# fukangl/SMG-multimodal-grasping

Hardware: AMD Instinct MI355X
Metric: affordance fwd+bwd passes/sec (16-rot 224^2 RGB-D) (higher is better)
Workload: dtype f32; 1 GPU; 16 rot x 224^2 (S=640): fwd + Huber + bwd + Adam per GPU per step; reinforcement_net style 0; 17 trunk passes; fp32; leg=headline, rotations=16, input_size=640, parallelism=dp1

## Files before the change

### smg-multimodal-grasping_amd/csrc/backward.hip

```cpp
#include "engine.h"

int do_backward(smg_engine* e, const smg_net* net, const float* dq, hipStream_t st, int phases, bool elem_head) {
    if (!e->have_fwd) return fail(-22, "smg_backward without a preceding smg_forward");
    if (!net->grads) return fail(-22, "net.grads is NULL");
    if (phases == 2 && !e->bw_phase0_done)
        return fail(-22, "smg_backward_phase(1) must follow smg_backward_phase(0) of the same forward");
    if ((phases & 1) && e->bw_phase0_done)
        return fail(-22, "smg_backward / smg_backward_phase(0) while the second half of a two-phase backward is still due (run phase 1 or a new forward)");
    const Layout& L = *e->L;
    const TrunkRef& T = L.trunk[e->f_trunk];
    const HeadRef& Hd = L.head[e->f_head];
    const int NS = e->f_streams, NP = e->f_pairs;
    const float* P = net->params;
    float* Gr = net->grads;
    const Plane p4 = e->p_blk[3];
    const bool ph_a = phases & 1, ph_b = phases & 2;
    if (ph_a) {
        for (int r = 0; r < kStatRep; ++r) HIP_OK(hipMemsetAsync(e->bstat + (size_t)r * kStatRepStride, 0, 2 * e->bstat_span * sizeof(double), st));
    }
    const bool split16 = e->prec == 0 && kSplitOp == 3;
    if (ph_a && split16) HIP_OK(hipMemsetAsync(e->gamax, 0, (size_t)e->gamax_words * sizeof(unsigned), st));
    const hipStream_t s2 = (e->prof || e->serialize) ? st : e->side;
    auto fork = [&](hipEvent_t ev) -> int {
        HIP_OK(hipEventRecord(ev, st));
// ... 183 lines not shown
            };
            PREC_DISPATCH(e, if (int rc = go(PTAG)) return rc);
        }
        return 0;
    };
    auto debug_stop = [&]() -> int {
        launch_reduce2(e, s2, tiles.drain());
        HIP_OK(hipEventRecord(e->ev_end, s2));
        HIP_OK(hipStreamWaitEvent(st, e->ev_end, 0));
        HIP_OK(hipMemsetAsync(e->dbscr, 0, (size_t)kDbRep * e->db_total * sizeof(float), st));
        if (int rc = walk_status(e)) return rc;
        e->have_fwd = false; e->bw_phase0_done = false; e->prof_stage = -1;
        return 0;
    };
    const bool pooled_tail = e->prec == 0 && e->f_stem1 && !e->stem_plane_tail && (NS > 4 || e->deterministic);
    for (int b = ph_a ? 3 : 0; b >= (ph_b ? 0 : 1); --b) {
        e->prof_stage = b;
        const Plane pl = e->p_blk[b];
        const int Ct = kBlockCtot[b];
        if (e->dbg_stop == b * 100 + 50) return debug_stop();
        if (b == 0 && pooled_tail) {
            StemMomArgs a;
            a.img = e->img4; a.pi = e->p_img; a.ps = e->p_stem; a.part = e->mom_part;
            a.tiles_x = stem_mom_tiles_x(e->p_stem); a.n_tiles = stem_mom_tiles(e->p_stem); a.tiles_per_wg = kMomTilesPerWg;
            if (fork(e->ev_misc)) return -5;
            e->prof_stage = -1;
            launch_kernel(e, stem_moments_kernel, dim3(e->mom_groups, NS), dim3(256), 0, s2, K_OTHER, 0, 0, false, a);
            launch_kernel(e, stem_moments_sum_kernel, dim3((kMomOut + 255) / 256, NS), dim3(256), 0, s2, K_OTHER, 0, 0, false,
                          (const float*)e->mom_part, e->mom_groups, e->mom);
            e->prof_stage = b;
// ... 117 lines not shown
                    p.ldg = kBottleneck; p.pa = pl; p.KA = kBottleneck; p.N = cs;
                    p.mbuf = e->X[b]; p.ldm = Ct;
                    p.msum = fsum(e, e->st_X[b]); p.msq = fsq(e, e->st_X[b]); p.mstride = Ct; p.mtab = stat_table(e, e->sx_tab[b], e->max_streams, Ct);
                    p.dst = e->G[b]; p.ldd = Ct;
                    p.o1 = b1(e, e->st_X[b]); p.o2 = b2(e, e->st_X[b]); p.ostride = Ct; p.rep_stride = e->db_total; p.eps = kEps;
                    launch_gemm(e, st, p, dim3(NS * pl.HWp / Cfg::BM, (cs + Cfg::BN - 1) / Cfg::BN), K_D1, 2.0 * NS * pl.HW * cs * kBottleneck * p.nseg,
                                ESZ(e) * NS * pl.HW * ((double)p.nseg * kBottleneck + 3.0 * cs));
                };
                PREC_DISPATCH(e, if (pl.HWp % 128 == 0) run(GemmCfg<128, 64, 32, 2, 2, 1, true>{}, PTAG); else run(CfgP64x64{}, PTAG));
            }
            if (e->dbg_stop == b * 100 + i) return debug_stop();
        }
        if (b > 0) {
            const Plane pp = e->p_blk[b - 1];
            const int Cp = kBlockCtot[b - 1], C0 = kBlockCin[b];
            {
                int chunk, cps;
                pick_chunk(pl, NS, (C0 / 128) * (Cp / 128), chunk, cps);
                auto go = [&](auto ptag) -> int {
                BwdWeightP<MC<CfgW128x128, decltype(ptag)::value>, W_POOL, C_IDENT, 1, true, decltype(ptag)::value> p{};
                p.gbuf = e->G[b]; p.ldg = Ct; p.gcoff = 0; p.xbuf = e->X[b]; p.ldx = Ct; p.xcoff = 0; p.pa = pl; p.MA = C0;
                p.xsum = fsum(e, e->st_X[b]); p.xsq = fsq(e, e->st_X[b]); p.xstride = Ct;
                p.s1 = b1(e, e->st_X[b]); p.s2 = b2(e, e->st_X[b]); p.sstride = Ct; p.scoff = 0; p.agamma = nullptr;
                p.bbuf = e->X[b - 1]; p.ldb = Cp; p.pb = pp; p.NB = Cp;
                p.bsum = fsum(e, e->st_X[b - 1]); p.bsq = fsq(e, e->st_X[b - 1]); p.bstride = Cp;
                p.bgamma = P + T.tnorm[b - 1].w; p.bbeta = P + T.tnorm[b - 1].b; p.eps = kEps;
                p.chunk = chunk; p.chunks_per_stream = cps; p.n_chunks = NS * cps;
                p.dw = Gr + T.tconv[b - 1].w; p.ldw_out = Cp;
                if (fork(e->ev_misc)) return -5;
                const dim3 grid(C0 / 128, Cp / 128, NS * cps);
                return launch_wgrad(e, s2, p, grid, K_TW, 2.0 * NS * pl.HW * Cp * C0,
                                    ESZ(e) * NS * (2.0 * pl.HW * C0 + (double)pp.HW * Cp), 1, C_IDENT, tiles, tiles.place_alone(wgrad_partial_floats(p, grid)));
                };
                PREC_DISPATCH(e, if (int rc = go(PTAG)) return rc);
            }
            if (pp.H != 2 * pl.H || pp.W != 2 * pl.W) {
                PREC_DISPATCH(e, launch_kernel(e, zero_uncovered_kernel<PREC>, dim3(256, NS), dim3(256), 0, st, K_OTHER, 0, 0, false,
                                               (void*)e->G[b - 1], Cp, pp, 2 * pl.H, 2 * pl.W, Cp));
            }
            {
                auto run = [&](auto tag, auto ptag) {
                using Cfg = MC<decltype(tag), decltype(ptag)::value>;
                BwdDataP<Cfg, false, E_UNPOOL, true, decltype(ptag)::value> p{};
                p.gbuf = e->G[b]; p.ldg = Ct; p.gcoff = 0; p.xbuf = e->X[b]; p.ldx = Ct; p.xcoff = 0; p.pa = pl; p.KA = C0;
                p.xsum = fsum(e, e->st_X[b]); p.xsq = fsq(e, e->st_X[b]); p.xstride = Ct;
                p.s1 = b1(e, e->st_X[b]); p.s2 = b2(e, e->st_X[b]); p.sstride = Ct; p.scoff = 0; p.agamma = nullptr;
                p.wp = e->packed_u + e->pk_td[b - 1]; p.K8tot = C0 / 8; p.ldn = Cp; p.wcol0 = 0; p.N = Cp;
                p.mbuf = e->X[b - 1]; p.ldm = Cp; p.mcoff = 0; p.pm = pp;
                p.msum = fsum(e, e->st_X[b - 1]); p.msq = fsq(e, e->st_X[b - 1]); p.mstride = Cp;
                p.egamma = P + T.tnorm[b - 1].w; p.ebeta = P + T.tnorm[b - 1].b;
                p.dst = e->G[b - 1]; p.ldd = Cp; p.dcoff = 0;
                p.o1 = b1(e, e->st_X[b - 1]); p.o2 = b2(e, e->st_X[b - 1]); p.ostride = Cp; p.ocoff = 0;
                p.dbeta = e->dbscr + e->db_toff[b - 1]; p.dgamma = e->dbscr + e->db_toff[b - 1] + Cp; p.rep_stride = e->db_total; p.eps = kEps;
                launch_gemm(e, st, p, dim3(NS * pl.HWp / Cfg::BM, Cp / Cfg::BN), K_TD, 2.0 * NS * pl.HW * Cp * C0,
                            ESZ(e) * NS * (2.0 * pl.HW * C0 + 2.0 * pp.HW * Cp));
            };
            PREC_DISPATCH(e, run(CfgP64x128{}, PTAG));
            }
        }
    }
    e->prof_stage = -1;
    if (ph_b && pooled_tail) {
        const Plane p1 = e->p_blk[0];
        StemTailArgs a;
        a.G1 = e->G[0]; a.X1 = e->X[0]; a.ld1 = kBlockCtot[0]; a.p1 = p1;
        a.xsum = fsum(e, e->st_X[0]); a.xsq = fsq(e, e->st_X[0]); a.xstride = kBlockCtot[0];
        a.SA = b1(e, e->st_X[0]); a.SB = b2(e, e->st_X[0]); a.sstride = kBlockCtot[0];
        a.argmax = e->argmax; a.stemv = e->stemv;
        a.ssum = fsum(e, e->st_stem); a.ssq = fsq(e, e->st_stem); a.ps = e->p_stem;
        a.gamma = P + T.norm0.w; a.eps = kEps;
        a.img = e->img4; a.pi = e->p_img;
        a.o1 = b1(e, e->st_stem); a.o2 = b2(e, e->st_stem);
// ... 77 lines not shown
```

### smg-multimodal-grasping_amd/csrc/elem.cuh

```cuda
#pragma once
#include "gemm.cuh"

namespace smg {

struct PrepArgs {
    const float* images_nchw;
    const double* heightmaps;
    int hm, pad, S;
    double mean, stdv;
    const int* stream_image;
    const float* stream_affine;
    const int* stream_rotated;
    float* img4;
    float* img1;
    int HWp;
    const double* masks;
    const int* stream_mask_a;
    const int* stream_mask_b;
};

__device__ __forceinline__ float lin_coord(int i, int S, float step) {
    return (i < S / 2) ? fmaf(step, (float)i, -1.f) : fmaf(-step, (float)(S - 1 - i), 1.f);
}

// ... 1232 lines not shown
#pragma unroll
    for (int o = 32; o > 0; o >>= 1) vmax = fmaxf(vmax, __shfl_xor(vmax, o));
    if ((t & 63) == 0) red[t >> 6] = vmax;
    __syncthreads();
    vmax = fmaxf(fmaxf(red[0], red[1]), fmaxf(red[2], red[3]));
    ActScale sc{1.f, 1.f};
    if (vmax > 0.f) sc = scale_of_max(__float_as_uint(vmax));
    if (t == 0) a.binv[(int64_t)n * (a.pl.HWp / kScaleBlock) + blockIdx.x] = sc.inv;
    char* ob = reinterpret_cast<char*>(a.out + d2_stream_units(n, a.pl.HWp));
#pragma unroll
    for (int k = 0; k < 8; ++k) {
        const Split4 s = split4<3>(mul4(gv[k], sc.s));
        const int64_t at = ((int64_t)(cs >> 1) * a.pl.HWp + r0 + 8 * k) * 16 + (cs & 1) * 8;
        *reinterpret_cast<uint2*>(ob + at) = s.p[0];
        *reinterpret_cast<uint2*>(ob + at + (int64_t)kD2K8 * a.pl.HWp * 16) = s.p[1];
    }
}

struct DbSegD { int64_t grad_off; int scr_off; int n; };
static __global__ void db_flush_kernel(const DbSegD* segs, float* scr, int rep_stride, int reps, float* grads,
                                       const double* stem1, const double* stem2, int ns, float* dbeta0, float* dgamma0) {
    if (blockIdx.y == gridDim.y - 1) {
        if (blockIdx.x == 0 && threadIdx.x < 128 && stem1) {
            const int q = threadIdx.x >> 6, c = threadIdx.x & 63;
            double v = 0.0;
            for (int n = 0; n < ns; ++n) v += stat_get(q ? stem2 : stem1, (int64_t)n * 64 + c);
            (q ? dgamma0 : dbeta0)[c] += (float)v;
        }
        return;
    }
// ... 238 lines not shown
```

### smg-multimodal-grasping_amd/csrc/engine.h

```cpp
#pragma once
#include <hip/hip_runtime.h>

#include <algorithm>
#include <cmath>
#include <cstdio>
#include <cstdlib>
#include <cstring>
#include <string>
#include <type_traits>
#include <vector>

#include "../../include/smg_hip.h"
#include "elem.cuh"
#include "scene.cuh"
#include "gemm.cuh"
#include "halo.cuh"
#include "ws.cuh"
#include "wsw.cuh"
#include "plan.h"

using namespace smg;

int smg_fail(int code, const std::string& msg);
static inline int fail(int code, const std::string& msg) { return smg_fail(code, msg); }
// ... 43 lines not shown

struct StatArr { int64_t off; int stride; };

struct smg_engine {
    int device = 0, S = 0, max_streams = 0, max_pairs = 0, head_out = 1;
    Plane p_img, p_stem, p_blk[4];
    int OH = 1, OW = 1;
    const Layout* L = nullptr;

    float* img4 = nullptr; float* stem = nullptr; float* X[4] = {}; float* Bt = nullptr;
    std::vector<int64_t> bt_off[4];
    unsigned char* argmax = nullptr;
    float* F = nullptr; float* H1 = nullptr;
    float* G[4] = {}; float* GS[kRing] = {}; float* D2[kRing] = {}; float* part = nullptr; int64_t part_floats = 0;
    float* DY2 = nullptr; float* D2S[kRing] = {};
    hipStream_t side = nullptr; hipEvent_t ev_gs[kRing] = {}, ev_d2[kRing] = {}, ev_side[kRing] = {}, ev_misc = nullptr, ev_end = nullptr; float* DY0 = nullptr; float* DH1 = nullptr; float* DF = nullptr;
    double* fstat = nullptr; int64_t fstat_span = 0;
    double* bstat = nullptr; int64_t bstat_span = 0;
    float* dbscr = nullptr; int db_total = 0; int db_off[4][24] = {}; int db_toff[3] = {}; struct DbSeg* d_dbseg = nullptr; int n_dbseg = 0;
    StatArr st_stem, st_X[4], st_F, st_H1; std::vector<StatArr> st_Bt[4];
    u32x4* packed_u = nullptr; int64_t packed_units = 0;
    float* packed_f = nullptr; int64_t packed_floats = 0;
    PackDesc* d_pack = nullptr; std::vector<PackDesc> h_pack[3]; std::vector<PackDesc> h_pack_head[3];
    int pack_stride = 0, bnupd_stride = 0, n_bnupd = 0;
    int64_t pk_conv0 = 0, pk_conv0_1 = 0, pk_head0 = 0, pk_hd0 = 0, pk_head1 = 0;
    std::vector<int64_t> pk_c1[4], pk_d1[4], pk_g3f[4], pk_g3d[4], pk_hf[4], pk_hd[4]; int64_t pk_t[3] = {}, pk_td[3] = {};
    int max_pack = 0;
    float* asc = nullptr; ActScaleDesc* d_asc = nullptr; int n_asc = 0;
    unsigned* gamax = nullptr; int64_t gamax_words = 0;
    float* stab = nullptr; int64_t stab_floats = 0;
    int64_t sx_tab[4] = {}, sb_tab[4][24] = {}, sf_tab = 0;
    BnUpdDesc* d_bnupd = nullptr;
    bool have_fwd = false; int f_trunk = 0, f_head = 0, f_streams = 0, f_pairs = 0;
    bool bw_phase0_done = false;
    bool f_dense_dq = false;
    int head_bwd = 0;
    bool f_stem1 = false;
    int* d_stream_image = nullptr; int* d_stream_rot = nullptr; int* d_pair_a = nullptr; int* d_pair_b = nullptr;
    int* d_seq_t = nullptr; int* d_seq_h = nullptr; int* d_user_ptr = nullptr; int* d_user_pair = nullptr; int* d_user_slot = nullptr;
    float* d_affine = nullptr;
    float* scene_val = nullptr; int* scene_idx = nullptr; int scene_tiles = 0;
    double* scene_lpart = nullptr;
    double* scene_gpart = nullptr; int* scene_cnt = nullptr;
    int* d_stage = nullptr; int* h_stage[2] = {}; hipEvent_t ev_stage[2] = {}; int stage_ints = 0, stage_turn = 0;
    int so_image = 0, so_rot = 0, so_pa = 0, so_pb = 0, so_seq_t = 0, so_seq_h = 0, so_uptr = 0, so_upair = 0, so_uslot = 0, so_aff = 0, so_ma = 0, so_mb = 0, so_adam = 0;
    bool capturing = false; int* h_stage_g = nullptr; hipEvent_t ev_graph = nullptr, ev_gin = nullptr; hipStream_t gstream = nullptr; struct StepGraph* step_graph = nullptr;
    int64_t workspace_bytes = 0;
    int n_cu = 256;
    int prec = 0;
    bool serialize = false;
    bool deterministic = false;
    bool generic3x3 = false, generic_c1 = false, generic_w1 = false, stem_plane_tail = false;
    float* stemv = nullptr; float* mom_part = nullptr; double* mom = nullptr; int mom_groups = 0;
    int dbg_stop = -1;
    float* dbg_gsnap = nullptr; int64_t dbg_gsnap_floats = 0;
    bool prof = false; std::vector<ProfRec> recs; std::vector<hipEvent_t> ev_pool;
    double prof_ms[5][K_COUNT] = {}; int64_t prof_n[5][K_COUNT] = {}; double prof_flops[5][K_COUNT] = {}; double prof_bytes[5][K_COUNT] = {}; int prof_stage = -1;
    int launch_rc = 0;
};

constexpr int kMomTilesPerWg = 8;
static inline int stem_mom_tiles_x(const Plane& ps) { return (ps.W + kMomT - 1) / kMomT; }
static inline int stem_mom_tiles(const Plane& ps) { return stem_mom_tiles_x(ps) * ((ps.H + kMomT - 1) / kMomT); }
static inline int stem_mom_groups(const Plane& ps) { return (stem_mom_tiles(ps) + kMomTilesPerWg - 1) / kMomTilesPerWg; }

static Plane make_plane(int H, int W) {
    Plane p; p.H = H; p.W = W; p.HW = H * W;
// ... 204 lines not shown
```

### smg-multimodal-grasping_amd/csrc/engine.hip

```cpp
#include "engine.h"

static thread_local std::string g_err;
int smg_fail(int code, const std::string& msg) { g_err = msg; return code; }

static int engine_build(smg_engine* e) {
    const Layout& L = *e->L;
    const int NS = e->max_streams, NP = e->max_pairs;
    const int S = e->S;
    const int H1 = (S - 1) / 2 + 1, H2 = (H1 - 1) / 2 + 1;
    e->p_img = make_plane(S, S);
    e->p_stem = make_plane(H1, H1);
    int h = H2;
    for (int b = 0; b < 4; ++b) { e->p_blk[b] = make_plane(h, h); h /= 2; }
    e->OH = e->OW = e->p_blk[3].H - kHeadKernel + 1;
    if (e->OH < 1) return fail(-22, "input_size too small for the 20x20 value head");

    if (getenv("SMG_SERIALIZE")) e->serialize = true;
    const int cross = getenv("SMG_CROSSCHECK") ? atoi(getenv("SMG_CROSSCHECK")) : 0;
    e->generic3x3 = cross & 1; e->generic_c1 = cross & 2; e->generic_w1 = cross & 4; e->stem_plane_tail = cross & 8;

    ALLOC(e->img4, (int64_t)NS * e->p_img.HWp * 4);
    ALLOC(e->stem, (int64_t)NS * e->p_stem.HWp * 64);
    ALLOC(e->DY0, (int64_t)NS * e->p_stem.HWp * 64);
    ALLOC(e->argmax, (int64_t)NS * e->p_blk[0].HWp * 64);
    e->stemv = e->DY0;
    e->mom_groups = stem_mom_groups(e->p_stem);
    ALLOC(e->mom_part, (int64_t)NS * e->mom_groups * kMomVals);
    ALLOC(e->mom, (int64_t)NS * kMomOut);
    int64_t bt_total = 0;
    for (int b = 0; b < 4; ++b) {
        ALLOC(e->X[b], (int64_t)NS * e->p_blk[b].HWp * kBlockCtot[b]);
        ALLOC(e->G[b], (int64_t)NS * e->p_blk[b].HWp * kBlockCtot[b]);
        for (int i = 0; i < kBlockLayers[b]; ++i) {
            e->bt_off[b].push_back(bt_total);
            bt_total += (int64_t)NS * e->p_blk[b].HWp * kBottleneck;
        }
    }
    ALLOC(e->Bt, bt_total);
    for (int k = 0; k < kRing; ++k) {
        ALLOC(e->D2[k], (int64_t)NS * e->p_blk[0].HWp * kBottleneck);
        ALLOC(e->GS[k], (int64_t)NS * e->p_blk[0].HWp * kGrowth);
        ALLOC(e->D2S[k], (int64_t)NS * (e->p_blk[0].HWp / kScaleBlock));
        HIP_OK(hipEventCreateWithFlags(&e->ev_gs[k], hipEventDisableTiming));
        HIP_OK(hipEventCreateWithFlags(&e->ev_d2[k], hipEventDisableTiming));
        HIP_OK(hipEventCreateWithFlags(&e->ev_side[k], hipEventDisableTiming));
    }
    ALLOC(e->DY2, (int64_t)NS * e->p_blk[0].HWp * kBottleneck);
    e->scene_tiles = (int)(((int64_t)(S / 2) * (S / 2) + kSceneTile - 1) / kSceneTile);
    ALLOC(e->scene_val, (int64_t)kSceneMaps * e->scene_tiles);
    ALLOC(e->scene_idx, (int64_t)kSceneMaps * e->scene_tiles);
    ALLOC(e->scene_lpart, (int64_t)kSceneMaps * e->OH * e->OW);
    ALLOC(e->scene_gpart, (int64_t)kSceneMaps * e->OH * e->OW * 3);
    ALLOC(e->scene_cnt, (int64_t)kSceneMaps * e->OH * e->OW);
    HIP_OK(hipEventCreateWithFlags(&e->ev_misc, hipEventDisableTiming));
    HIP_OK(hipEventCreateWithFlags(&e->ev_end, hipEventDisableTiming));
    HIP_OK(hipStreamCreateWithFlags(&e->side, hipStreamNonBlocking));
    e->part_floats = (int64_t)24 << 20;
    for (int b = 0; b < 4; ++b) {
        const Plane& pl = e->p_blk[b];
        for (int ts : {halo_tile(pl), 8})
            e->part_floats = std::max(e->part_floats, w3_partial_floats(w3_tiling(pl, ts, NS, INT64_MAX).groups, NS));
    }
    ALLOC(e->part, e->part_floats);
    ALLOC(e->F, (int64_t)NP * e->p_blk[3].HWp * 2 * kFeat);
    ALLOC(e->DF, (int64_t)NP * e->p_blk[3].HWp * 2 * kFeat);
    ALLOC(e->H1, (int64_t)NP * e->p_blk[3].HWp * kHeadMid);
    ALLOC(e->DH1, (int64_t)NP * e->p_blk[3].HWp * kHeadMid);

    int64_t off = 0;
    auto carve = [&](int n, int stride) { StatArr s{off, stride}; off += (int64_t)n * stride; return s; };
// ... 71 lines not shown
                int64_t g2 = 0, g3 = 0;
                const int64_t hf = add_units(v, d.c2.w, kGrowth, kBottleneck, PK_HF, 9 * kBottleneck, kGrowth, kSplitOp);
                const int64_t hd = add_units(v, d.c2.w, kGrowth, kBottleneck, PK_HD, 9 * kGrowth, kBottleneck, kSplitOp);
                if (e->generic3x3) {
                    g2 = add_units(v, d.c2.w, kGrowth, kBottleneck, PK_3F, 9 * kBottleneck, kGrowth, kSplitOp);
                    g3 = add_units(v, d.c2.w, kGrowth, kBottleneck, PK_3D, 9 * kGrowth, kBottleneck);
                }
                if (t == 0) {
                    e->pk_c1[b].push_back(a1); e->pk_d1[b].push_back(a1d);
                    e->pk_g3f[b].push_back(g2); e->pk_g3d[b].push_back(g3); e->pk_hf[b].push_back(hf); e->pk_hd[b].push_back(hd);
                }
            }
            if (b < 3) {
                e->pk_t[b] = add_units(v, T.tconv[b].w, T.tconv[b].cout, T.tconv[b].cin, PK_T1, T.tconv[b].cin, T.tconv[b].cout, kSplitOp);
                e->pk_td[b] = add_units(v, T.tconv[b].w, T.tconv[b].cout, T.tconv[b].cin, PK_D1, T.tconv[b].cout, T.tconv[b].cin);
            }
        }
    }
    const int64_t trunk_pku = pku, trunk_pkf = pkf;
    for (int hd = 0; hd < 3; ++hd) {
        pku = trunk_pku; pkf = trunk_pkf;
        const HeadRef& H = L.head[hd];
        std::vector<PackDesc>& v = e->h_pack_head[hd];
        e->pk_head0 = add_units(v, H.c0.w, kHeadMid, 2 * kFeat, PK_T1, 2 * kFeat, kHeadMid, kSplitOp);
        e->pk_hd0 = add_units(v, H.c0.w, kHeadMid, 2 * kFeat, PK_D1, kHeadMid, 2 * kFeat);
        e->pk_head1 = add_f32(v, H.c1.w, e->head_out, kHeadMid, PK_HEAD, H.c1.count());
    }
    e->packed_units = pku + 4096;
    e->packed_floats = pkf;
    ALLOC(e->packed_u, e->packed_units);
// ... 186 lines not shown
    {
        int cus = 0;
        if (hipDeviceGetAttribute(&cus, hipDeviceAttributeMultiprocessorCount, device) == hipSuccess && cus > 0) e->n_cu = cus;
    }
    int r = engine_build(e);
    if (r) { smg_engine_destroy(e); return r; }
    *out = e;
    return 0;
}

void smg_engine_destroy(smg_engine* e) {
    if (!e) return;
    (void)hipSetDevice(e->device);
    (void)hipDeviceSynchronize();
    void* ptrs[] = {e->img4, e->stem, e->DY0, e->argmax, e->X[0], e->X[1], e->X[2], e->X[3], e->G[0], e->G[1], e->G[2], e->G[3],
                    e->Bt, e->DY2, e->part, e->F, e->DF, e->H1, e->DH1, e->fstat, e->bstat, e->dbscr, e->d_dbseg, e->asc, e->d_asc, e->gamax, e->packed_u, e->packed_f, e->stab, e->d_pack, e->d_bnupd,
                    e->d_stage, e->scene_val, e->scene_idx, e->scene_lpart, e->scene_gpart, e->scene_cnt, e->mom_part, e->mom};
    for (void* p : ptrs) if (p) (void)hipFree(p);
    if (e->dbg_gsnap) (void)hipFree(e->dbg_gsnap);
    step_graph_drop(e);
    if (e->h_stage_g) (void)hipHostFree(e->h_stage_g);
    if (e->ev_graph) (void)hipEventDestroy(e->ev_graph);
    if (e->ev_gin) (void)hipEventDestroy(e->ev_gin);
    if (e->gstream) (void)hipStreamDestroy(e->gstream);
    for (int k = 0; k < 2; ++k) { if (e->h_stage[k]) (void)hipHostFree(e->h_stage[k]); if (e->ev_stage[k]) (void)hipEventDestroy(e->ev_stage[k]); }
    for (int k = 0; k < kRing; ++k) {
        if (e->D2[k]) (void)hipFree(e->D2[k]);
        if (e->GS[k]) (void)hipFree(e->GS[k]);
        if (e->D2S[k]) (void)hipFree(e->D2S[k]);
        if (e->ev_gs[k]) (void)hipEventDestroy(e->ev_gs[k]); if (e->ev_d2[k]) (void)hipEventDestroy(e->ev_d2[k]); if (e->ev_side[k]) (void)hipEventDestroy(e->ev_side[k]);
    }
    if (e->ev_misc) (void)hipEventDestroy(e->ev_misc);
    if (e->ev_end) (void)hipEventDestroy(e->ev_end);
    if (e->side) (void)hipStreamDestroy(e->side);
    for (auto& r : e->recs) { (void)hipEventDestroy(r.a); (void)hipEventDestroy(r.b); }
    for (auto ev : e->ev_pool) (void)hipEventDestroy(ev);
    delete e;
}

int64_t smg_engine_workspace_bytes(const smg_engine* e) { return e ? e->workspace_bytes : 0; }

int smg_engine_geometry(const smg_engine* e, int H[6], int HWp[6]) {
    if (!e) return fail(-22, "engine is NULL");
    const Plane* pl[6] = {&e->p_img, &e->p_stem, &e->p_blk[0], &e->p_blk[1], &e->p_blk[2], &e->p_blk[3]};
    for (int i = 0; i < 6; ++i) { H[i] = pl[i]->H; HWp[i] = pl[i]->HWp; }
    return 0;
}

// ... 576 lines not shown
```

### smg-multimodal-grasping_amd/csrc/gemm.cuh

```cuda
#pragma once
#include <hip/hip_runtime.h>
#include <stdint.h>

#include <type_traits>

#include "wgrad_plan.h"

namespace smg {
constexpr int kDmaFlyDgrad = 2, kDmaFlyGroup = 1;
constexpr int kPdFwdSmall = 3;
constexpr int kPdFwdBig = 2;
constexpr int kPdDgrad = 2;
constexpr int kPdDgradBig = 2;
constexpr int kPdWgrad = 3;
constexpr int kPdDgradGroup = 1;
constexpr int kFwdBigMinWaves = 3;
}

namespace smg {

typedef float f32x16 __attribute__((ext_vector_type(16)));
typedef __bf16 bf16x8 __attribute__((ext_vector_type(8)));
typedef short s16x4 __attribute__((ext_vector_type(4)));
typedef unsigned u32x4 __attribute__((ext_vector_type(4)));
// ... 1167 lines not shown
    int N;
    const void* mbuf; int ldm; int mcoff; Plane pm;
    const double* msum; const double* msq; int mstride; StatTab mtab;
    const float* egamma; const float* ebeta;
    void* dst; int ldd; int dcoff;
    double* o1; double* o2; int ostride; int ocoff;
    float* dbeta; float* dgamma; int rep_stride;
    float eps;
    TileMap tm;
    static constexpr int kSwizzle = 1;
    static constexpr int kPrefetch = (Cfg::TM * Cfg::TN <= 2) ? kPdDgrad : kPdDgradBig;
    static constexpr int kDmaFly = kAUnit ? kDmaFlyDgrad : 0;
    static constexpr bool kSegmented = false;
    static constexpr bool kHasPrologue = true;
    static constexpr bool kEarlyFetch = EMODE != E_UNPOOL;
    static constexpr int kMinWaves = (PREC == 0 && EMODE == E_UNPOOL) ? 3 : 1;

    static constexpr bool kFast = !SHIFT3 && !AFF;
    static constexpr bool kEarly = EMODE != E_UNPOOL;
    static constexpr bool kWide = GT::size == 2;
    struct Ctx {
        int n, m0, n0; bool whole;
        float ginv[2];
        float xv[(kEarly && !kWide) ? Cfg::TM : 1][(kEarly && !kWide) ? Cfg::TN : 1][16];
        float gold[(kEarly && !kWide && EMODE == E_ACCUM) ? Cfg::TM : 1][(kEarly && !kWide && EMODE == E_ACCUM) ? Cfg::TN : 1][16];
        rawq_t<XT> xq[(kEarly && kWide) ? Cfg::TM : 1][(kEarly && kWide) ? Cfg::TN : 1][4];
        rawq_t<GT> gq[(kEarly && kWide && EMODE == E_ACCUM) ? Cfg::TM : 1][(kEarly && kWide && EMODE == E_ACCUM) ? Cfg::TN : 1][4];
    };
    struct ARow { int y, x; bool valid; unsigned off; };
    struct DRow {};
    using KPrm = KPrm0;
    using KFin = KPrm0;
    __device__ KPrm k_fetch(const Ctx&, int, int) const { return KPrm{}; }
    __device__ KFin k_finish(const Ctx&, const KPrm&, int, int, const float*) const { return KFin{}; }

    __host__ __device__ int param_floats() const { return 4 * KA + 5 * Cfg::BN; }

    __device__ void d_init(const Ctx&, DRow&, int) const {}
    __device__ void d_next(const Ctx&, DRow&) const {}
    __device__ bool init_ctx(Ctx& c, const VBlock& vb) const {
        int mt = vb.x, nt = vb.y;
        if (tm.nM && !tile_decode(tm, vb.x, mt, nt)) return false;
        c.m0 = sgpr(mt * Cfg::BM);
        c.n0 = sgpr(nt * Cfg::BN);
        c.n = sgpr(c.m0 / pa.HWp);
        const int pbase = c.m0 - c.n * pa.HWp;
        if (pbase >= pa.HW) return false;
        c.whole = kEarly && pbase + Cfg::BM <= pa.HW && (c.n0 + Cfg::BN <= N || (N & 31) == 0);
        c.ginv[0] = c.ginv[1] = 1.f;
        if constexpr (kOp == 3) {
            static_assert(Cfg::BM == kScaleBlock || (Cfg::BM == 2 * kScaleBlock && Cfg::WM == 2), "a wave's rows lie in one scale block");
            const float* bi = binv + (int64_t)c.n * (pa.HWp / kScaleBlock) + pbase / kScaleBlock;
            const float wi = pack_inv_scale(wp);
            c.ginv[0] = bi[0] * wi;
            c.ginv[1] = (Cfg::BM > kScaleBlock ? bi[1] : bi[0]) * wi;
        }
        return true;
    }
    __device__ UnitSrc a_unit_src(const Ctx& c, int kt, int piece, int k8, int row) const {
        return UnitSrc{static_cast<const u32x4*>(gbuf) + d2_stream_units(c.n, pa.HWp), kWholeBuf,
                       16u * (unsigned)((piece * kD2K8 + k8) * pa.HWp + row), 16u * (unsigned)(kt * Cfg::K8 * pa.HWp + (c.m0 - c.n * pa.HWp))};
    }
    __device__ u32x4 a_unit(const Ctx& c, int kt, int piece, int k8, int row) const {
        const UnitSrc u = a_unit_src(c, kt, piece, k8, row);
        return bload_u4(u.base, u.bytes, u.voff, u.soff);
    }
    __device__ u32x4 a_unit_d(const Ctx&, int, int, int, int) const { return u32x4{}; }
    __device__ void early_fetch(Ctx& c) const {
        if constexpr (kEarly) {
            if (c.whole) {
                const int t = threadIdx.x, lane = t & 63, wmn = (t >> 6) % (Cfg::WM * Cfg::WN), l31 = lane & 31, half = lane >> 5;
                const int wm0 = (wmn / Cfg::WN) * Cfg::TM * 32, wn0 = (wmn % Cfg::WN) * Cfg::TN * 32;
                if constexpr (kWide) {
    #pragma unroll
                    for (int i = 0; i < Cfg::TM; ++i)
    #pragma unroll
// ... 31 lines not shown
        }
    }
    __device__ void init_params(const Ctx& c, float* sp) const {
        const double inv = 1.0 / (double)pa.HW;
        for (int k = threadIdx.x; xbuf && k < KA; k += 256) {
            float mean, invstd;
            bn_moments(xsum, xsq, (int64_t)c.n * xstride + xcoff + k, inv, eps, mean, invstd);
            const float g = agamma ? agamma[k] : 1.f;
            const float q1 = (float)(stat_get(s1, (int64_t)c.n * sstride + scoff + k) * inv);
            const float q2 = (float)(stat_get(s2, (int64_t)c.n * sstride + scoff + k) * inv);
            sp[k] = g * invstd;
            sp[KA + k] = q1;
            sp[2 * KA + k] = mean;
            sp[3 * KA + k] = invstd * q2;
        }
        float* ep = sp + 4 * KA;
        const double minv = 1.0 / (double)pm.HW;
        for (int j = threadIdx.x; j < Cfg::BN; j += 256) {
            const int col = c.n0 + j;
            float mean = 0.f, invstd = 0.f, g = 0.f, b = 0.f;
            if (col < N) {
                tab_or_moments(mtab, c.n, mcoff + col, msum, msq, (int64_t)c.n * mstride + mcoff + col, minv, eps, mean, invstd);
                g = egamma[col];
                b = ebeta[col];
            }
            ep[j] = g * invstd;
            ep[Cfg::BN + j] = b;
            ep[2 * Cfg::BN + j] = mean;
            ep[3 * Cfg::BN + j] = invstd;
            ep[4 * Cfg::BN + j] = g;
        }
// ... 47 lines not shown
        if (!xbuf) return o.v[0];
        return affine2(o.v[0], o.v[1], sp + a_chan(kt, q), KA);
    }
    __device__ ARaw a_fetch_d(const Ctx&, const DRow&, int, int, int) const { return ARaw{}; }
    __device__ UnitSrc b_unit_src(const Ctx& c, int kt, int piece, int k8, int r) const {
        return UnitSrc{wp, kWholeBuf, 16u * (unsigned)((piece * K8tot + k8) * ldn + r), 16u * (unsigned)(kt * Cfg::K8 * ldn + wcol0 + c.n0)};
    }
    __device__ BRaw b_unit(const Ctx& c, int kt, int piece, int k8, int r) const {
        const UnitSrc u = b_unit_src(c, kt, piece, k8, r);
        return bload_u4(u.base, u.bytes, u.voff, u.soff);
    }
    __device__ u32x4 b_unit_xform(const Ctx&, const BRaw& o, int) const { return o; }
    __device__ void epilogue(const Ctx& c, f32x16 (&acc)[Cfg::TM][Cfg::TN], float* smem, float* sp, bool active) const {
        const int t = threadIdx.x, lane = t & 63, wmn = (t >> 6) % (Cfg::WM * Cfg::WN), l31 = lane & 31, half = lane >> 5;
        const int wm0 = (wmn / Cfg::WN) * Cfg::TM * 32, wn0 = (wmn % Cfg::WN) * Cfg::TN * 32;
        const float* ep = sp + 4 * KA;
#ifdef SMG_TRACE_EPI
        unsigned long long* etr = (g_smg_trace && threadIdx.x == 0) ? g_smg_trace + 8 * (size_t)blockIdx.x : nullptr;
        if (etr) etr[0] = smg_stamp();
#endif
        float v[2][Cfg::TN];
#pragma unroll
        for (int j = 0; j < Cfg::TN; ++j) v[0][j] = v[1][j] = 0.f;
        if constexpr (kOp == 3) {
            const float gi = wm0 >= kScaleBlock ? c.ginv[1] : c.ginv[0];
#pragma unroll
            for (int i = 0; i < Cfg::TM; ++i)
#pragma unroll
                for (int j = 0; j < Cfg::TN; ++j)
#pragma unroll
                    for (int r = 0; r < 16; ++r) acc[i][j][r] *= gi;
// ... 78 lines not shown
                                o[k] = pg_[k] * dy;
                                s0[k] += dy;
                                s1[k] += dy * ((xv4[k] - pm_[k]) * pi_[k]);
                            }
                            stq<GT>(dst, (pix0 + (d >> 1) * pm.W + (d & 1)) * ldd + dcoff + c.n0 + cq0, make_float4(o[0], o[1], o[2], o[3]));
                        }
                        quad_transpose4(s0[0], s0[1], s0[2], s0[3]);
                        quad_transpose4(s1[0], s1[1], s1[2], s1[3]);
                        v[0][j] += (s0[0] + s0[1]) + (s0[2] + s0[3]);
                        v[1][j] += (s1[0] + s1[1]) + (s1[2] + s1[3]);
                    }
            } else
#pragma unroll
            for (int i = 0; i < Cfg::TM; ++i) {
                constexpr int NL = (EMODE == E_UNPOOL) ? 4 : 1;
                constexpr int RB = (EMODE == E_UNPOOL) ? 8 : 16;
#pragma unroll
                for (int rb = 0; rb < 16; rb += RB) {
                    float xv[RB][NL], gold[RB];
                    int pix0[RB];
                    bool ok[RB];
#pragma unroll
                    for (int q = 0; q < RB; ++q) {
                        const int r = rb + q;
                        const int row = SMG_ACC_ROW(wm0, i, r, half);
                        const int p = pbase + row;
                        ok[q] = active && p < pa.HW && cok;
                        gold[q] = 0.f;
                        if constexpr (EMODE == E_UNPOOL) {
                            const int y = p / pa.W, x = p - y * pa.W;
                            pix0[q] = c.n * pm.HWp + (2 * y) * pm.W + 2 * x;
// ... 432 lines not shown
        if (etr) { etr[3] = smg_stamp(); asm volatile("s_waitcnt vmcnt(0)" ::: "memory"); etr[4] = smg_stamp(); }
#endif
    }
};

enum { W_ONE = 0, W_THREE = 1, W_POOL = 2, W_STEM = 3, W_STEM1 = 4 };

template <class Cfg_, int BMODE, int CMAP, int PD_ = kPdWgrad, bool AFF = true, int PREC = 0, bool F32IO_ = false>
struct BwdWeightP {
    using Cfg = Cfg_;
    static_assert(!Cfg::AT, "weight-gradient form");
    static constexpr bool F32IO = F32IO_ || BMODE == 3 || BMODE == 4;
    using GT = typename std::conditional<F32IO, e_f32, grd_t<PREC>>::type;
    using XT = typename std::conditional<F32IO, e_f32, act_t<PREC>>::type;
    static_assert(GT::size == XT::size, "one slot geometry");
    static constexpr int kOp = (!AFF && BMODE == 0) ? bwd_op(PREC) : bwd_op_plain(PREC), kAE = 16 / GT::size, kBE = 16 / XT::size, GSZ = GT::size, XSZ = XT::size;
    static constexpr bool kARawCopy = !AFF && kAE == 8;
    static constexpr bool kAUnit = !AFF && BMODE == 0 && kOp == 3;
    static constexpr bool kH = kOp == 3;
    const float* binv;
    const float* basc;
    const void* gbuf; int ldg; int gcoff;
    const void* xbuf; int ldx; int xcoff;
    Plane pa; int MA;
    const double* xsum; const double* xsq; int xstride;
    const double* s1; const double* s2; int sstride; int scoff;
    const float* agamma;
    const void* bbuf; int ldb; Plane pb; int NB;
    const double* bsum; const double* bsq; int bstride; StatTab btab;
    const float* bgamma; const float* bbeta;
    float eps;
    int chunk, chunks_per_stream, n_chunks;
    float* dw; int ldw_out;
// ... 44 lines not shown
        c.m0 = sgpr((tile % gx) * Cfg::BM);
        c.n0 = sgpr((tile / gx) * Cfg::BN);
        c.tap = sgpr(z / n_chunks);
        const int ci = z - c.tap * n_chunks;
        c.n = sgpr(ci / chunks_per_stream);
        c.p0 = sgpr((ci - c.n * chunks_per_stream) * chunk);
        if (c.p0 >= pa.HW) return false;
        int len = pa.HWp - c.p0;
        len = len < chunk ? len : chunk;
        c.kt = sgpr(len / Cfg::BK);
        c.cur_inv = 1.f;
        if constexpr (kAUnit) c.cur_inv = binv[(int64_t)c.n * (pa.HWp / kScaleBlock) + c.p0 / kScaleBlock];
        return true;
    }
    __device__ u32x4 a_unit_d(const Ctx& c, int kt, int piece, int k8, int kr) const {
        return bload_u4(static_cast<const u32x4*>(gbuf) + d2_stream_units(c.n, pa.HWp), 16u * (unsigned)(2 * kD2K8 * pa.HWp),
                        16u * (unsigned)((piece * kD2K8 + k8) * pa.HWp + kr), 16u * (unsigned)(c.p0 + kt * Cfg::BK));
    }
    __device__ u32x4 a_unit(const Ctx&, int, int, int, int) const { return u32x4{}; }
    __device__ void k_hook(Ctx& c, int kt, f32x16 (&acc)[Cfg::TM][Cfg::TN], const float* sp) const {
        if constexpr (kAUnit) {
            const int nx = (kt + 1) * Cfg::BK;
            if (nx % kScaleBlock || kt + 1 >= c.kt) return;
            const float inv = sp[kInvAt + nx / kScaleBlock];
            if (inv != c.cur_inv) {
                const float f = c.cur_inv * __uint_as_float((254u << 23) - __float_as_uint(inv));
#pragma unroll
                for (int i = 0; i < Cfg::TM; ++i)
#pragma unroll
                    for (int j = 0; j < Cfg::TN; ++j)
#pragma unroll
                        for (int r = 0; r < 16; ++r) acc[i][j][r] *= f;
// ... 263 lines not shown
```

Before: 64.54 passes/s.

## Precompute transition-layer gradient units once and share across wgrad and dgrad

Adds a trans_units_kernel that applies the BN-backward affine to the transition gradient once per block, computes per-row-block scales, and writes split 16-bit unit tiles. The pooled transition weight-gradient and unpool data-gradient GEMMs then read these precomputed units instead of each recomputing the affine from fp32 G/X. This replaces reading fp32 G and X twice with one extra kernel pass plus a compact buffer. It adds an event to guard reuse of the TU buffer across blocks and raises min waves for the non-affine unpool path.

```diff
diff --git a/smg-multimodal-grasping_amd/csrc/backward.hip b/smg-multimodal-grasping_amd/csrc/backward.hip
--- a/smg-multimodal-grasping_amd/csrc/backward.hip
+++ b/smg-multimodal-grasping_amd/csrc/backward.hip
@@ -221,6 +221,7 @@
         return 0;
     };
     const bool pooled_tail = e->prec == 0 && e->f_stem1 && !e->stem_plane_tail && (NS > 4 || e->deterministic);
+    bool tu_busy = false;
     for (int b = ph_a ? 3 : 0; b >= (ph_b ? 0 : 1); --b) {
         e->prof_stage = b;
         const Plane pl = e->p_blk[b];
@@ -368,14 +369,31 @@
         if (b > 0) {
             const Plane pp = e->p_blk[b - 1];
             const int Cp = kBlockCtot[b - 1], C0 = kBlockCin[b];
+            const bool t_units = split16 && !e->trans_on_the_fly && NS > 4;
+            if (t_units) {
+                if (tu_busy) HIP_OK(hipStreamWaitEvent(st, e->ev_tu, 0));
+                TransUnitsArgs a{};
+                a.g = e->G[b]; a.x = e->X[b]; a.ld = Ct; a.pl = pl; a.xtab = stat_table(e, e->sx_tab[b], e->max_streams, Ct);
+                a.s1 = b1(e, e->st_X[b]); a.s2 = b2(e, e->st_X[b]); a.sstride = Ct;
+                a.out = reinterpret_cast<u32x4*>(e->TU); a.binv = e->TUS;
+                const dim3 grid(pl.HWp / kScaleBlock, NS);
+                const double bytes = 4.0 * NS * pl.HW * 3 * C0;
+                if (C0 == 128) launch_kernel(e, trans_units_kernel<128>, grid, dim3(256), 0, st, K_OTHER, 0, bytes, false, a);
+                else if (C0 == 256) launch_kernel(e, trans_units_kernel<256>, grid, dim3(512), 0, st, K_OTHER, 0, bytes, false, a);
+                else launch_kernel(e, trans_units_kernel<512>, grid, dim3(1024), 0, st, K_OTHER, 0, bytes, false, a);
+            }
             {
                 int chunk, cps;
                 pick_chunk(pl, NS, (C0 / 128) * (Cp / 128), chunk, cps);
-                auto go = [&](auto ptag) -> int {
-                BwdWeightP<MC<CfgW128x128, decltype(ptag)::value>, W_POOL, C_IDENT, 1, true, decltype(ptag)::value> p{};
-                p.gbuf = e->G[b]; p.ldg = Ct; p.gcoff = 0; p.xbuf = e->X[b]; p.ldx = Ct; p.xcoff = 0; p.pa = pl; p.MA = C0;
+                auto go = [&](auto ptag, auto afftag) -> int {
+                constexpr bool AFF = decltype(afftag)::value;
+                BwdWeightP<MC<CfgW128x128, decltype(ptag)::value>, W_POOL, C_IDENT, 1, AFF, decltype(ptag)::value> p{};
+                p.pa = pl; p.MA = C0;
+                if constexpr (AFF) {
+                p.gbuf = e->G[b]; p.ldg = Ct; p.gcoff = 0; p.xbuf = e->X[b]; p.ldx = Ct; p.xcoff = 0;
                 p.xsum = fsum(e, e->st_X[b]); p.xsq = fsq(e, e->st_X[b]); p.xstride = Ct;
                 p.s1 = b1(e, e->st_X[b]); p.s2 = b2(e, e->st_X[b]); p.sstride = Ct; p.scoff = 0; p.agamma = nullptr;
+                } else { p.gbuf = e->TU; p.xbuf = nullptr; p.binv = e->TUS; p.basc = asc_trans(e, b - 1); }
                 p.bbuf = e->X[b - 1]; p.ldb = Cp; p.pb = pp; p.NB = Cp;
                 p.bsum = fsum(e, e->st_X[b - 1]); p.bsq = fsq(e, e->st_X[b - 1]); p.bstride = Cp;
                 p.bgamma = P + T.tnorm[b - 1].w; p.bbeta = P + T.tnorm[b - 1].b; p.eps = kEps;
@@ -386,20 +404,28 @@
                 return launch_wgrad(e, s2, p, grid, K_TW, 2.0 * NS * pl.HW * Cp * C0,
                                     ESZ(e) * NS * (2.0 * pl.HW * C0 + (double)pp.HW * Cp), 1, C_IDENT, tiles, tiles.place_alone(wgrad_partial_floats(p, grid)));
                 };
-                PREC_DISPATCH(e, if (int rc = go(PTAG)) return rc);
+                if (t_units) {
+                    if (int rc = go(std::integral_constant<int, 0>{}, std::false_type{})) return rc;
+                    HIP_OK(hipEventRecord(e->ev_tu, s2));
+                    tu_busy = true;
+                } else PREC_DISPATCH(e, if (int rc = go(PTAG, std::true_type{})) return rc);
             }
             if (pp.H != 2 * pl.H || pp.W != 2 * pl.W) {
                 PREC_DISPATCH(e, launch_kernel(e, zero_uncovered_kernel<PREC>, dim3(256, NS), dim3(256), 0, st, K_OTHER, 0, 0, false,
                                                (void*)e->G[b - 1], Cp, pp, 2 * pl.H, 2 * pl.W, Cp));
             }
             {
-                auto run = [&](auto tag, auto ptag) {
+                auto run = [&](auto tag, auto ptag, auto afftag) {
                 using Cfg = MC<decltype(tag), decltype(ptag)::value>;
-                BwdDataP<Cfg, false, E_UNPOOL, true, decltype(ptag)::value> p{};
-                p.gbuf = e->G[b]; p.ldg = Ct; p.gcoff = 0; p.xbuf = e->X[b]; p.ldx = Ct; p.xcoff = 0; p.pa = pl; p.KA = C0;
+                constexpr bool AFF = decltype(afftag)::value;
+                BwdDataP<Cfg, false, E_UNPOOL, AFF, decltype(ptag)::value> p{};
+                p.pa = pl; p.KA = C0;
+                if constexpr (AFF) {
+                p.gbuf = e->G[b]; p.ldg = Ct; p.gcoff = 0; p.xbuf = e->X[b]; p.ldx = Ct; p.xcoff = 0;
                 p.xsum = fsum(e, e->st_X[b]); p.xsq = fsq(e, e->st_X[b]); p.xstride = Ct;
                 p.s1 = b1(e, e->st_X[b]); p.s2 = b2(e, e->st_X[b]); p.sstride = Ct; p.scoff = 0; p.agamma = nullptr;
-                p.wp = e->packed_u + e->pk_td[b - 1]; p.K8tot = C0 / 8; p.ldn = Cp; p.wcol0 = 0; p.N = Cp;
+                } else { p.gbuf = e->TU; p.xbuf = nullptr; p.binv = e->TUS; }
+                p.wp = e->packed_u + (AFF ? e->pk_td[b - 1] : e->pk_tdu[b - 1]); p.K8tot = C0 / 8; p.ldn = Cp; p.wcol0 = 0; p.N = Cp;
                 p.mbuf = e->X[b - 1]; p.ldm = Cp; p.mcoff = 0; p.pm = pp;
                 p.msum = fsum(e, e->st_X[b - 1]); p.msq = fsq(e, e->st_X[b - 1]); p.mstride = Cp;
                 p.egamma = P + T.tnorm[b - 1].w; p.ebeta = P + T.tnorm[b - 1].b;
@@ -409,7 +435,8 @@
                 launch_gemm(e, st, p, dim3(NS * pl.HWp / Cfg::BM, Cp / Cfg::BN), K_TD, 2.0 * NS * pl.HW * Cp * C0,
                             ESZ(e) * NS * (2.0 * pl.HW * C0 + 2.0 * pp.HW * Cp));
             };
-            PREC_DISPATCH(e, run(CfgP64x128{}, PTAG));
+            if (t_units) run(CfgP64x128{}, std::integral_constant<int, 0>{}, std::false_type{});
+            else PREC_DISPATCH(e, run(CfgP64x128{}, PTAG, std::true_type{}));
             }
         }
     }
diff --git a/smg-multimodal-grasping_amd/csrc/elem.cuh b/smg-multimodal-grasping_amd/csrc/elem.cuh
--- a/smg-multimodal-grasping_amd/csrc/elem.cuh
+++ b/smg-multimodal-grasping_amd/csrc/elem.cuh
@@ -1270,6 +1270,65 @@
         const int64_t at = ((int64_t)(cs >> 1) * a.pl.HWp + r0 + 8 * k) * 16 + (cs & 1) * 8;
         *reinterpret_cast<uint2*>(ob + at) = s.p[0];
         *reinterpret_cast<uint2*>(ob + at + (int64_t)kD2K8 * a.pl.HWp * 16) = s.p[1];
+    }
+}
+
+struct TransUnitsArgs {
+    const float* g; const float* x; int ld;
+    Plane pl;
+    StatTab xtab;
+    const double* s1; const double* s2; int sstride;
+    u32x4* out; float* binv;
+};
+template <int C>
+static __global__ __launch_bounds__(2 * C) void trans_units_kernel(const TransUnitsArgs a) {
+    constexpr int NW = 2 * C / 64, K8 = C / 8;
+    __shared__ float prm[4 * C];
+    __shared__ float red[NW];
+    const int n = blockIdx.y, t = threadIdx.x;
+    const int cs = t >> 3, rr = t & 7;
+    const int r0 = blockIdx.x * kScaleBlock + rr;
+    float4 gv[8], xv[8];
+#pragma unroll
+    for (int k = 0; k < 8; ++k) {
+        const int r = r0 + 8 * k;
+        const int64_t pix = (int64_t)n * a.pl.HWp + (r < a.pl.HW ? r : 0);
+        gv[k] = ld4(a.g + pix * a.ld + 4 * cs);
+        xv[k] = ld4(a.x + pix * a.ld + 4 * cs);
+    }
+    if (t < C) {
+        const double inv = 1.0 / (double)a.pl.HW;
+        const float invstd = a.xtab.invstd[(int64_t)n * a.xtab.ld + t];
+        prm[t] = invstd;
+        prm[C + t] = (float)(stat_get(a.s1, (int64_t)n * a.sstride + t) * inv);
+        prm[2 * C + t] = a.xtab.mean[(int64_t)n * a.xtab.ld + t];
+        prm[3 * C + t] = invstd * (float)(stat_get(a.s2, (int64_t)n * a.sstride + t) * inv);
+    }
+    __syncthreads();
+    float vmax = 0.f;
+#pragma unroll
+    for (int k = 0; k < 8; ++k) {
+        const float4 o = r0 + 8 * k < a.pl.HW ? affine2(gv[k], xv[k], prm + 4 * cs, C) : zero4();
+        gv[k] = o;
+        vmax = fmaxf(fmaxf(vmax, fmaxf(fabsf(o.x), fabsf(o.y))), fmaxf(fabsf(o.z), fabsf(o.w)));
+    }
+#pragma unroll
+    for (int o = 32; o > 0; o >>= 1) vmax = fmaxf(vmax, __shfl_xor(vmax, o));
+    if ((t & 63) == 0) red[t >> 6] = vmax;
+    __syncthreads();
+    vmax = red[0];
+#pragma unroll
+    for (int w = 1; w < NW; ++w) vmax = fmaxf(vmax, red[w]);
+    ActScale sc{1.f, 1.f};
+    if (vmax > 0.f) sc = scale_of_max(__float_as_uint(vmax));
+    if (t == 0) a.binv[(int64_t)n * (a.pl.HWp / kScaleBlock) + blockIdx.x] = sc.inv;
+    char* ob = reinterpret_cast<char*>(a.out + (int64_t)n * 2 * K8 * a.pl.HWp);
+#pragma unroll
+    for (int k = 0; k < 8; ++k) {
+        const Split4 s = split4<3>(mul4(gv[k], sc.s));
+        const int64_t at = ((int64_t)(cs >> 1) * a.pl.HWp + r0 + 8 * k) * 16 + (cs & 1) * 8;
+        *reinterpret_cast<uint2*>(ob + at) = s.p[0];
+        *reinterpret_cast<uint2*>(ob + at + (int64_t)K8 * a.pl.HWp * 16) = s.p[1];
     }
 }
 
diff --git a/smg-multimodal-grasping_amd/csrc/engine.h b/smg-multimodal-grasping_amd/csrc/engine.h
--- a/smg-multimodal-grasping_amd/csrc/engine.h
+++ b/smg-multimodal-grasping_amd/csrc/engine.h
@@ -81,7 +81,8 @@
     float* F = nullptr; float* H1 = nullptr;
     float* G[4] = {}; float* GS[kRing] = {}; float* D2[kRing] = {}; float* part = nullptr; int64_t part_floats = 0;
     float* DY2 = nullptr; float* D2S[kRing] = {};
-    hipStream_t side = nullptr; hipEvent_t ev_gs[kRing] = {}, ev_d2[kRing] = {}, ev_side[kRing] = {}, ev_misc = nullptr, ev_end = nullptr; float* DY0 = nullptr; float* DH1 = nullptr; float* DF = nullptr;
+    float* TU = nullptr; float* TUS = nullptr;
+    hipStream_t side = nullptr; hipEvent_t ev_gs[kRing] = {}, ev_d2[kRing] = {}, ev_side[kRing] = {}, ev_misc = nullptr, ev_end = nullptr, ev_tu = nullptr; float* DY0 = nullptr; float* DH1 = nullptr; float* DF = nullptr;
     double* fstat = nullptr; int64_t fstat_span = 0;
     double* bstat = nullptr; int64_t bstat_span = 0;
     float* dbscr = nullptr; int db_total = 0; int db_off[4][24] = {}; int db_toff[3] = {}; struct DbSeg* d_dbseg = nullptr; int n_dbseg = 0;
@@ -91,7 +92,7 @@
     PackDesc* d_pack = nullptr; std::vector<PackDesc> h_pack[3]; std::vector<PackDesc> h_pack_head[3];
     int pack_stride = 0, bnupd_stride = 0, n_bnupd = 0;
     int64_t pk_conv0 = 0, pk_conv0_1 = 0, pk_head0 = 0, pk_hd0 = 0, pk_head1 = 0;
-    std::vector<int64_t> pk_c1[4], pk_d1[4], pk_g3f[4], pk_g3d[4], pk_hf[4], pk_hd[4]; int64_t pk_t[3] = {}, pk_td[3] = {};
+    std::vector<int64_t> pk_c1[4], pk_d1[4], pk_g3f[4], pk_g3d[4], pk_hf[4], pk_hd[4]; int64_t pk_t[3] = {}, pk_td[3] = {}, pk_tdu[3] = {};
     int max_pack = 0;
     float* asc = nullptr; ActScaleDesc* d_asc = nullptr; int n_asc = 0;
     unsigned* gamax = nullptr; int64_t gamax_words = 0;
@@ -117,7 +118,7 @@
     int prec = 0;
     bool serialize = false;
     bool deterministic = false;
-    bool generic3x3 = false, generic_c1 = false, generic_w1 = false, stem_plane_tail = false;
+    bool generic3x3 = false, generic_c1 = false, generic_w1 = false, stem_plane_tail = false, trans_on_the_fly = false;
     float* stemv = nullptr; float* mom_part = nullptr; double* mom = nullptr; int mom_groups = 0;
     int dbg_stop = -1;
     float* dbg_gsnap = nullptr; int64_t dbg_gsnap_floats = 0;
diff --git a/smg-multimodal-grasping_amd/csrc/engine.hip b/smg-multimodal-grasping_amd/csrc/engine.hip
--- a/smg-multimodal-grasping_amd/csrc/engine.hip
+++ b/smg-multimodal-grasping_amd/csrc/engine.hip
@@ -17,7 +17,7 @@
 
     if (getenv("SMG_SERIALIZE")) e->serialize = true;
     const int cross = getenv("SMG_CROSSCHECK") ? atoi(getenv("SMG_CROSSCHECK")) : 0;
-    e->generic3x3 = cross & 1; e->generic_c1 = cross & 2; e->generic_w1 = cross & 4; e->stem_plane_tail = cross & 8;
+    e->generic3x3 = cross & 1; e->generic_c1 = cross & 2; e->generic_w1 = cross & 4; e->stem_plane_tail = cross & 8; e->trans_on_the_fly = cross & 16;
 
     ALLOC(e->img4, (int64_t)NS * e->p_img.HWp * 4);
     ALLOC(e->stem, (int64_t)NS * e->p_stem.HWp * 64);
@@ -46,6 +46,15 @@
         HIP_OK(hipEventCreateWithFlags(&e->ev_side[k], hipEventDisableTiming));
     }
     ALLOC(e->DY2, (int64_t)NS * e->p_blk[0].HWp * kBottleneck);
+    {
+        int64_t tu = 0, tus = 0;
+        for (int b = 1; b < 4; ++b) {
+            tu = std::max(tu, (int64_t)NS * e->p_blk[b].HWp * kBlockCin[b]);
+            tus = std::max(tus, (int64_t)NS * (e->p_blk[b].HWp / kScaleBlock));
+        }
+        ALLOC(e->TU, tu);
+        ALLOC(e->TUS, tus);
+    }
     e->scene_tiles = (int)(((int64_t)(S / 2) * (S / 2) + kSceneTile - 1) / kSceneTile);
     ALLOC(e->scene_val, (int64_t)kSceneMaps * e->scene_tiles);
     ALLOC(e->scene_idx, (int64_t)kSceneMaps * e->scene_tiles);
@@ -54,6 +63,7 @@
     ALLOC(e->scene_cnt, (int64_t)kSceneMaps * e->OH * e->OW);
     HIP_OK(hipEventCreateWithFlags(&e->ev_misc, hipEventDisableTiming));
     HIP_OK(hipEventCreateWithFlags(&e->ev_end, hipEventDisableTiming));
+    HIP_OK(hipEventCreateWithFlags(&e->ev_tu, hipEventDisableTiming));
     HIP_OK(hipStreamCreateWithFlags(&e->side, hipStreamNonBlocking));
     e->part_floats = (int64_t)24 << 20;
     for (int b = 0; b < 4; ++b) {
@@ -155,6 +165,7 @@
             if (b < 3) {
                 e->pk_t[b] = add_units(v, T.tconv[b].w, T.tconv[b].cout, T.tconv[b].cin, PK_T1, T.tconv[b].cin, T.tconv[b].cout, kSplitOp);
                 e->pk_td[b] = add_units(v, T.tconv[b].w, T.tconv[b].cout, T.tconv[b].cin, PK_D1, T.tconv[b].cout, T.tconv[b].cin);
+                e->pk_tdu[b] = add_units(v, T.tconv[b].w, T.tconv[b].cout, T.tconv[b].cin, PK_D1, T.tconv[b].cout, T.tconv[b].cin, kSplitOp);
             }
         }
     }
@@ -371,7 +382,7 @@
     (void)hipSetDevice(e->device);
     (void)hipDeviceSynchronize();
     void* ptrs[] = {e->img4, e->stem, e->DY0, e->argmax, e->X[0], e->X[1], e->X[2], e->X[3], e->G[0], e->G[1], e->G[2], e->G[3],
-                    e->Bt, e->DY2, e->part, e->F, e->DF, e->H1, e->DH1, e->fstat, e->bstat, e->dbscr, e->d_dbseg, e->asc, e->d_asc, e->gamax, e->packed_u, e->packed_f, e->stab, e->d_pack, e->d_bnupd,
+                    e->Bt, e->DY2, e->TU, e->TUS, e->part, e->F, e->DF, e->H1, e->DH1, e->fstat, e->bstat, e->dbscr, e->d_dbseg, e->asc, e->d_asc, e->gamax, e->packed_u, e->packed_f, e->stab, e->d_pack, e->d_bnupd,
                     e->d_stage, e->scene_val, e->scene_idx, e->scene_lpart, e->scene_gpart, e->scene_cnt, e->mom_part, e->mom};
     for (void* p : ptrs) if (p) (void)hipFree(p);
     if (e->dbg_gsnap) (void)hipFree(e->dbg_gsnap);
@@ -389,6 +400,7 @@
     }
     if (e->ev_misc) (void)hipEventDestroy(e->ev_misc);
     if (e->ev_end) (void)hipEventDestroy(e->ev_end);
+    if (e->ev_tu) (void)hipEventDestroy(e->ev_tu);
     if (e->side) (void)hipStreamDestroy(e->side);
     for (auto& r : e->recs) { (void)hipEventDestroy(r.a); (void)hipEventDestroy(r.b); }
     for (auto ev : e->ev_pool) (void)hipEventDestroy(ev);
diff --git a/smg-multimodal-grasping_amd/csrc/gemm.cuh b/smg-multimodal-grasping_amd/csrc/gemm.cuh
--- a/smg-multimodal-grasping_amd/csrc/gemm.cuh
+++ b/smg-multimodal-grasping_amd/csrc/gemm.cuh
@@ -1205,7 +1205,7 @@
     static constexpr bool kSegmented = false;
     static constexpr bool kHasPrologue = true;
     static constexpr bool kEarlyFetch = EMODE != E_UNPOOL;
-    static constexpr int kMinWaves = (PREC == 0 && EMODE == E_UNPOOL) ? 3 : 1;
+    static constexpr int kMinWaves = (PREC == 0 && EMODE == E_UNPOOL) ? (AFF ? 3 : 4) : 1;
 
     static constexpr bool kFast = !SHIFT3 && !AFF;
     static constexpr bool kEarly = EMODE != E_UNPOOL;
@@ -1225,7 +1225,8 @@
     __device__ KPrm k_fetch(const Ctx&, int, int) const { return KPrm{}; }
     __device__ KFin k_finish(const Ctx&, const KPrm&, int, int, const float*) const { return KFin{}; }
 
-    __host__ __device__ int param_floats() const { return 4 * KA + 5 * Cfg::BN; }
+    __host__ __device__ int ep_at() const { return (kAUnit && EMODE == E_UNPOOL) ? 0 : 4 * KA; }
+    __host__ __device__ int param_floats() const { return ep_at() + 5 * Cfg::BN; }
 
     __device__ void d_init(const Ctx&, DRow&, int) const {}
     __device__ void d_next(const Ctx&, DRow&) const {}
@@ -1249,8 +1250,9 @@
         return true;
     }
     __device__ UnitSrc a_unit_src(const Ctx& c, int kt, int piece, int k8, int row) const {
-        return UnitSrc{static_cast<const u32x4*>(gbuf) + d2_stream_units(c.n, pa.HWp), kWholeBuf,
-                       16u * (unsigned)((piece * kD2K8 + k8) * pa.HWp + row), 16u * (unsigned)(kt * Cfg::K8 * pa.HWp + (c.m0 - c.n * pa.HWp))};
+        const int k8n = EMODE == E_UNPOOL ? KA >> 3 : kD2K8;
+        return UnitSrc{static_cast<const u32x4*>(gbuf) + (int64_t)c.n * 2 * k8n * pa.HWp, kWholeBuf,
+                       16u * (unsigned)((piece * k8n + k8) * pa.HWp + row), 16u * (unsigned)(kt * Cfg::K8 * pa.HWp + (c.m0 - c.n * pa.HWp))};
     }
     __device__ u32x4 a_unit(const Ctx& c, int kt, int piece, int k8, int row) const {
         const UnitSrc u = a_unit_src(c, kt, piece, k8, row);
@@ -1312,7 +1314,7 @@
             sp[2 * KA + k] = mean;
             sp[3 * KA + k] = invstd * q2;
         }
-        float* ep = sp + 4 * KA;
+        float* ep = sp + ep_at();
         const double minv = 1.0 / (double)pm.HW;
         for (int j = threadIdx.x; j < Cfg::BN; j += 256) {
             const int col = c.n0 + j;
@@ -1390,7 +1392,7 @@
     __device__ void epilogue(const Ctx& c, f32x16 (&acc)[Cfg::TM][Cfg::TN], float* smem, float* sp, bool active) const {
         const int t = threadIdx.x, lane = t & 63, wmn = (t >> 6) % (Cfg::WM * Cfg::WN), l31 = lane & 31, half = lane >> 5;
         const int wm0 = (wmn / Cfg::WN) * Cfg::TM * 32, wn0 = (wmn % Cfg::WN) * Cfg::TN * 32;
-        const float* ep = sp + 4 * KA;
+        const float* ep = sp + ep_at();
 #ifdef SMG_TRACE_EPI
         unsigned long long* etr = (g_smg_trace && threadIdx.x == 0) ? g_smg_trace + 8 * (size_t)blockIdx.x : nullptr;
         if (etr) etr[0] = smg_stamp();
@@ -1499,7 +1501,7 @@
 #pragma unroll
             for (int i = 0; i < Cfg::TM; ++i) {
                 constexpr int NL = (EMODE == E_UNPOOL) ? 4 : 1;
-                constexpr int RB = (EMODE == E_UNPOOL) ? 8 : 16;
+                constexpr int RB = (EMODE == E_UNPOOL) ? (kAUnit ? 4 : 8) : 16;
 #pragma unroll
                 for (int rb = 0; rb < 16; rb += RB) {
                     float xv[RB][NL], gold[RB];
@@ -1962,9 +1964,10 @@
     using GT = typename std::conditional<F32IO, e_f32, grd_t<PREC>>::type;
     using XT = typename std::conditional<F32IO, e_f32, act_t<PREC>>::type;
     static_assert(GT::size == XT::size, "one slot geometry");
-    static constexpr int kOp = (!AFF && BMODE == 0) ? bwd_op(PREC) : bwd_op_plain(PREC), kAE = 16 / GT::size, kBE = 16 / XT::size, GSZ = GT::size, XSZ = XT::size;
+    static constexpr bool kUnitMode = BMODE == W_ONE || BMODE == W_POOL;
+    static constexpr int kOp = (!AFF && kUnitMode) ? bwd_op(PREC) : bwd_op_plain(PREC), kAE = 16 / GT::size, kBE = 16 / XT::size, GSZ = GT::size, XSZ = XT::size;
     static constexpr bool kARawCopy = !AFF && kAE == 8;
-    static constexpr bool kAUnit = !AFF && BMODE == 0 && kOp == 3;
+    static constexpr bool kAUnit = !AFF && kUnitMode && kOp == 3;
     static constexpr bool kH = kOp == 3;
     const float* binv;
     const float* basc;
@@ -2039,8 +2042,9 @@
         return true;
     }
     __device__ u32x4 a_unit_d(const Ctx& c, int kt, int piece, int k8, int kr) const {
-        return bload_u4(static_cast<const u32x4*>(gbuf) + d2_stream_units(c.n, pa.HWp), 16u * (unsigned)(2 * kD2K8 * pa.HWp),
-                        16u * (unsigned)((piece * kD2K8 + k8) * pa.HWp + kr), 16u * (unsigned)(c.p0 + kt * Cfg::BK));
+        const int k8n = BMODE == W_POOL ? MA >> 3 : kD2K8, k80 = BMODE == W_POOL ? c.m0 >> 3 : 0;
+        return bload_u4(static_cast<const u32x4*>(gbuf) + (int64_t)c.n * 2 * k8n * pa.HWp, 16u * (unsigned)(2 * k8n * pa.HWp),
+                        16u * (unsigned)((piece * k8n + k80 + k8) * pa.HWp + kr), 16u * (unsigned)(c.p0 + kt * Cfg::BK));
     }
     __device__ u32x4 a_unit(const Ctx&, int, int, int, int) const { return u32x4{}; }
     __device__ void k_hook(Ctx& c, int kt, f32x16 (&acc)[Cfg::TM][Cfg::TN], const float* sp) const {
```

Result: no change. 64.86 passes/s (median of 6 runs) (+0.5%).
